# itmo153277/JoshUpscale

Hardware: AMD Instinct MI355X
Metric: frames/sec 480x270->1920x1080 recurrent SR (higher is better)
Workload: dtype bf16

## Files before the change

joshupscale_amd/csrc/c_api.cpp:

```cpp

#include "joshupscale_amd.h"
#ifdef JU_TEST_HOOKS
#include "joshupscale_amd_test.h"
#endif

#include <cstdio>
#include <cstring>
#include <fstream>
#include <ios>
#include <new>
#include <stdexcept>
#include <string>
#include <vector>

#include "engine.h"
#include "fp8.h"
#include "graphics.h"
#include "log.h"
#include "model.h"
#include "tiled.h"

struct ju_runtime {
	std::unique_ptr<ju::Engine> engine;
};
// ... 1452 lines not shown
}

int ju_debug_e4m3(const float *values, unsigned char *codes, size_t count) {
	return guarded([&] {
		if (count && (!values || !codes)) throw std::invalid_argument("ju_debug_e4m3: null buffer");
		for (size_t i = 0; i < count; ++i) codes[i] = ju::e4m3FromFloat(values[i]);
	});
}

}
namespace {

constexpr int kDebugAxisMax = 4096;

struct DebugRefuse {
	const char *hook;
	[[noreturn]] void operator()(const std::string &why) const { throw std::invalid_argument(std::string(hook) + ": " + why); }
};

bool misaligned(const void *p, std::uintptr_t a) { return reinterpret_cast<std::uintptr_t>(p) % a != 0; }

ju::DType debugDType(const DebugRefuse &refuse, int dtype) {
	if (dtype != JU_DTYPE_F16 && dtype != JU_DTYPE_BF16) refuse("dtype must be JU_DTYPE_F16 or JU_DTYPE_BF16");
	return dtype == JU_DTYPE_F16 ? ju::kF16 : ju::kBF16;
}

void debugActivation(const DebugRefuse &refuse, int act, float slope) {
	if (act < 0 || act > 2) refuse("an activation code outside 0 .. 2");
	if (act == 2 && !(slope >= 0.0f && slope <= 1.0f)) refuse("a LeakyReLU slope outside [0, 1]");
}

ju::DevPlan debugPlan(const DebugRefuse &refuse, const ju_debug_plan &p, ju::PlanLog *log) {
	if (p.flow_tile < 0 || p.res_block < 0 || p.res_block > 2 || p.conv_stages < -1 || p.conv_stages > 2 || p.splitk_rows < 0 ||
	    p.splitk_blocks < 0 || p.splitk_blocks > 2 || p.conv_nb < 0 || p.conv_nb > 2 || p.conv_rw < 0 || p.conv_rw > 2) {
		refuse("a plan field out of range");
	}
	ju::DevPlan plan;
	plan.flowTile = p.flow_tile;
	plan.resBlock = p.res_block;
	plan.convStages = p.conv_stages;
	plan.splitkRows = p.splitk_rows;
	plan.splitkBlocks = p.splitk_blocks;
	plan.convNb = p.conv_nb;
	plan.convRw = p.conv_rw;
	plan.log = log;
	return plan;
}

void debugPlanText(const ju::PlanLog &log, char *dst, std::size_t capacity) {
	if (dst == nullptr || capacity == 0) return;
	const std::string text = log.text();
	const std::size_t n = std::min(text.size(), capacity - 1);
	std::memcpy(dst, text.data(), n);
	dst[n] = '\0';
}

ju::DeviceBuffer debugPackWeights(const float *w, int taps, int cinReal, int cinPadded, int cout, int nb, ju::DType dt) {
	ju::FoldedConv conv;
	conv.taps = taps;
	conv.cin = cinReal;
	conv.cout = cout;
	conv.w.assign(w, w + static_cast<std::size_t>(taps) * cinReal * cout);
	std::vector<int> cinMap(static_cast<std::size_t>(cinPadded), -1);
	for (int c = 0; c < cinReal; ++c) cinMap[static_cast<std::size_t>(c)] = c;
	const std::vector<std::uint16_t> packed = ju::packConvWeights(conv, cinMap, nb, dt);
	ju::DeviceBuffer dev(packed.size() * 2);
	dev.upload(packed.data(), packed.size() * 2);
	return dev;
}

ju::DeviceBuffer debugUploadBias(const float *bias, int cout) {
	ju::DeviceBuffer dev(static_cast<std::size_t>(cout) * 4);
	dev.upload(bias, static_cast<std::size_t>(cout) * 4);
	return dev;
}

void debugPitch(const DebugRefuse &refuse, int pitch, int width, const char *what) {
// ... 362 lines not shown
```

joshupscale_amd/csrc/dev_switch.cpp:

```cpp
#include "dev_switch.h"

#ifdef JU_TEST_HOOKS
#include <cstddef>
#include <cstdlib>
#endif

namespace ju {

#ifdef JU_TEST_HOOKS
const char *devSwitch(Dev which) {
	static const char *const kNames[] = {
	    "JU_TAIL", "JU_PACK", "JU_POOL", "JU_UPSAMPLE", "JU_FLOW_CONV", "JU_TOWER", "JU_CALIBRATE", "JU_FLOW", "JU_DIRECT",
	    "JU_DIRECT_GRAPH", "JU_SYNC_SPIN_US", "JU_TRACE_STEPS", "JU_TRACE_NOSYNC", "JU_RES_BLOCK", "JU_FLOW_TILE",
	    "JU_FLOW_WIDE", "JU_WAVE_PRIO", "JU_CONV_DBUF", "JU_TOWER_FAST", "JU_FP8_GRID", "JU_FP8_BLOCK", "JU_SPLITK_PLAN",
	    "JU_CONV_TILE",
	};
	static_assert(sizeof(kNames) / sizeof(kNames[0]) == static_cast<std::size_t>(Dev::Count),
	    "kNames must name every switch of Dev, in its order");
	const int i = static_cast<int>(which);
	if (i < 0 || i >= static_cast<int>(Dev::Count)) return nullptr;
	return std::getenv(kNames[i]);
}
bool devSwitchesExist() {
	return true;
}
#else
const char *devSwitch(Dev) {
	return nullptr;
}
bool devSwitchesExist() {
	return false;
}
#endif

}
```

joshupscale_amd/csrc/dev_switch.h:

```cpp
#pragma once

namespace ju {

enum class Dev : int {
	Tail,
	Pack,
	Pool,
	Upsample,
	FlowConv,
	Tower,
	Calibrate,
	Flow,
	Direct,
	DirectGraph,
	SyncSpinUs,
	TraceSteps,
	TraceNoSync,
	ResBlock,
	FlowTile,
	FlowWide,
	WavePrio,
	ConvDbuf,
	TowerFast,
	Fp8Grid,
	Fp8Block,
	SplitKPlan,
	ConvTile,
	Count
};

const char *devSwitch(Dev which);
bool devSwitchesExist();

}
```

joshupscale_amd/csrc/engine.cpp:

```cpp
#include "engine.h"

#include <cstdio>

#include <algorithm>
#include <atomic>
#include <cstdlib>
#include <cstring>
#include <memory>
#include <mutex>
#include <sstream>
#include <stdexcept>

#include "dev_switch.h"
#include "fp8.h"
#include "graphics.h"
#include "log.h"

namespace ju {

namespace {
thread_local int g_DryLaunches = 0;
}
bool launchesAreDry() { return g_DryLaunches > 0; }
DryLaunchScope::DryLaunchScope() { ++g_DryLaunches; }
// ... 175 lines not shown
			throw std::invalid_argument("fp8 tower needs a 64-filter generator with at least one residual block");
		}
		m_Fp8Tower = true;
		dt = kF16;
	}
	if (dt != kF16 && dt != kBF16) throw std::invalid_argument("Unsupported compute dtype");
	m_DType = static_cast<DType>(dt);
	readSwitches();
	planFlowUnits();
	buildWeights(model);
	setUpResidentTowers();
	allocateBuffers(model);
	buildProgram(0);
	buildProgram(1);
	bindStaging();
	warmUpAndCapture();
}

namespace {
bool switchIs(Dev which, const char *word) {
	const char *v = devSwitch(which);
	return v && std::string(v) == word;
}
}

void Engine::readSwitches() {
	m_FusedTail = !switchIs(Dev::Tail, "split");
	m_TailInTower = !switchIs(Dev::Tail, "fused") && !switchIs(Dev::Tail, "split");
	m_PackInBlock = !switchIs(Dev::Pack, "split");
	m_FusedPool = !switchIs(Dev::Pool, "split");
	m_FusedUpsample = !switchIs(Dev::Upsample, "split");
	m_FlowFused = !switchIs(Dev::FlowConv, "generic");
	if (const char *e = devSwitch(Dev::FlowTile)) m_Plan.flowTile = std::atoi(e);
	if (const char *e = devSwitch(Dev::ResBlock)) m_Plan.resBlock = std::string(e) == "plain" ? 1 : (std::string(e) == "tile" ? 2 : 0);
	if (const char *e = devSwitch(Dev::ConvDbuf)) m_Plan.convStages = (e[0] >= '0' && e[0] <= '2') ? e[0] - '0' : -1;
	if (const char *e = devSwitch(Dev::SplitKPlan)) {
		m_Plan.splitkRows = std::atoi(e);
		if (const char *x = std::strchr(e, 'x')) m_Plan.splitkBlocks = std::atoi(x + 1);
	}
	if (const char *e = devSwitch(Dev::ConvTile)) {
		m_Plan.convNb = std::atoi(e);
		if (const char *x = std::strchr(e, 'x')) m_Plan.convRw = std::atoi(x + 1);
	}
	if (devSwitchesExist()) m_Plan.log = &m_PlanLog;
	const char *direct = devSwitch(Dev::Direct);
	m_PreferDirect = !(direct && direct[0] == '0');
	if (const char *retry = std::getenv("JU_RESIDENT_RETRY")) m_RetryBase = static_cast<unsigned>(std::atoi(retry));
	const char *directGraph = devSwitch(Dev::DirectGraph);
	m_DirectGraph = !(directGraph && directGraph[0] == '0');
	if (const char *spin = devSwitch(Dev::SyncSpinUs)) m_SpinUs = static_cast<unsigned>(std::atoi(spin));
	if (const char *la = std::getenv("JU_LOOKAHEAD")) m_BatchMax = std::min(std::max(std::atoi(la), 1), kFlowBatchMax);
}

bool Engine::setUpResidentTower(ResidentTower *t, bool wanted, int H, int W, int cus, bool leaky) {
	const bool on = wanted && residentTowerGeometry(H, W, cus, &t->GX, &t->GY, &t->RH);
	if (on) {
		t->w = DeviceBuffer(t->hostW.size() * 2);
		t->w.upload(t->hostW.data(), t->hostW.size() * 2);
		t->b = DeviceBuffer(t->hostB.size() * 4);
		t->b.upload(t->hostB.data(), t->hostB.size() * 4);
		const bool eightBit = m_Fp8Tower && t == &m_GenTower;
		t->mail = DeviceBuffer(eightBit ? residentMailboxBytes8(t->GX, t->GY, leaky) : residentMailboxBytes(t->GX, t->GY, leaky));
		t->flags = DeviceBuffer(residentCounterBytes(t->GX, t->GY));
	}
	t->hostW.clear();
	t->hostW.shrink_to_fit();
// ... 712 lines not shown
```

joshupscale_amd/csrc/flow_block_common.h:

```cpp
#pragma once

#include "kernel_common.h"

namespace ju {

void launchResBlockPersistent(DType dt, const FlowBlockLaunch &q, hipStream_t stream);

namespace {

constexpr int kFbW = 34;
constexpr int kFbOutW = 30;

__device__ __forceinline__ void fbGlds16(const void *g, void *l) {
	__builtin_amdgcn_global_load_lds((const __attribute__((address_space(1))) void *)g,
	    (__attribute__((address_space(3))) void *)l, 16, 0, 0);
}

template <int PB>
__device__ __forceinline__ unsigned fbSwz(unsigned col) {
	if constexpr (PB == 256) return col & 15u;
	else if constexpr (PB == 128) return (col >> 1) & 7u;
	else if constexpr (PB == 64) return (col >> 2) & 3u;
	else return (col >> 3) & 1u;
}

template <typename T, int KS, int PB>
struct FbPair {
	static constexpr int RS = kFbW * PB;
	static constexpr int NMAC = 3 * KS;

	template <int J>
	static __device__ __forceinline__ void rd(Vec8<T> &dst, unsigned a) {
		asm volatile("ds_read_b128 %0, %1 offset:%2" : "=v"(dst) : "v"(a), "n"(RS * J));
	}
	template <int ROT = 0>
	static __device__ __forceinline__ void issue(Vec8<T> (&fb)[4], unsigned rowAddr,
	    const unsigned (&colOff)[3], const unsigned (&colSwz)[3], int hh, int m, int j) {
		const int dx = m / KS, ks = m % KS;
		const unsigned a = rowAddr + colOff[dx] + ((static_cast<unsigned>(ks * 2 + hh) ^ colSwz[dx]) << 4);
		if (j == 0) rd<(0 + ROT) % 4>(fb[0], a);
		else if (j == 1) rd<(1 + ROT) % 4>(fb[1], a);
		else if (j == 2) rd<(2 + ROT) % 4>(fb[2], a);
		else rd<(3 + ROT) % 4>(fb[3], a);
	}
	template <int N>
	static __device__ __forceinline__ void waitLgkm() {
		static_assert(N >= 0 && N <= 4, "lgkmcnt");
		if constexpr (N == 4) asm volatile("s_waitcnt lgkmcnt(4)" ::: "memory");
		else if constexpr (N == 3) asm volatile("s_waitcnt lgkmcnt(3)" ::: "memory");
		else if constexpr (N == 2) asm volatile("s_waitcnt lgkmcnt(2)" ::: "memory");
		else if constexpr (N == 1) asm volatile("s_waitcnt lgkmcnt(1)" ::: "memory");
		else asm volatile("s_waitcnt lgkmcnt(0)" ::: "memory");
	}

	template <int ROT = 0>
	static __device__ __forceinline__ void run(unsigned rowAddr, const unsigned (&colOff)[3],
	    const unsigned (&colSwz)[3], int hh, const Vec8<T> (&w)[9 * KS], f32x16 (&acc)[2]) {
		Vec8<T> fb[2][4];
		asm volatile("s_waitcnt lgkmcnt(0)" ::: "memory");
		__builtin_amdgcn_sched_barrier(0);
#pragma unroll
		for (int j = 0; j < 4; ++j) issue<ROT>(fb[0], rowAddr, colOff, colSwz, hh, 0, j);
#pragma unroll
		for (int m = 0; m < NMAC; ++m) {
			const int set = m & 1;
			const bool more = m + 1 < NMAC;
			const int dx = m / KS, ks = m % KS;
#pragma unroll
			for (int k = 0; k < 6; ++k) {
				const int dy = k >> 1, r = k & 1;
				const int need = r + dy;
				const bool fresh = k == 0 || k == 1 || k == 3 || k == 5;
				if (fresh) {
					const int allowed = (3 - need) + (more ? (k < 4 ? k : 4) : 0);
					if (allowed >= 4) waitLgkm<4>();
					else if (allowed == 3) waitLgkm<3>();
					else if (allowed == 2) waitLgkm<2>();
					else if (allowed == 1) waitLgkm<1>();
					else waitLgkm<0>();
					__builtin_amdgcn_sched_barrier(0);
				}
				acc[r] = mfma32(w[(dy * 3 + dx) * KS + ks], fb[set][need], acc[r]);
				if (more && k < 4) issue<ROT>(fb[set ^ 1], rowAddr, colOff, colSwz, hh, m + 1, k);
				__builtin_amdgcn_sched_barrier(0);
			}
		}
	}
};


__device__ __forceinline__ float fbActS(int act, float slope) {
	return act == 1 ? 0.0f : (act == 2 ? slope : 1.0f);
}
__device__ __forceinline__ float fbAct(float v, float s) {
	return v < 0.0f ? v * s : v;
}

__device__ __forceinline__ float fbSwapPair(float v) {
	return __builtin_bit_cast(float, __builtin_amdgcn_mov_dpp(__builtin_bit_cast(int, v), 0xB1, 0xF, 0xF, true));
}

}

}
```

joshupscale_amd/csrc/flow_kernels.hip:

```cpp
#include "flow_block_common.h"

namespace ju {

namespace {

struct FlowBlockParams {
	const void *in;
	const void *w1;
	const float *b1;
	const void *w2;
	const float *b2;
	void *out;
	int H, W;
	int inPitch, outPitch;
	int act1, act2;
	float slope;
	int skip;
	int prio;
	const void *packPrev;
	void *packOut;
	int frameH, frameW, padTop, padLeft, numInputs;
	const unsigned *sums;
	long inItem, outItem;
	const std::uint8_t *frames[kFlowBatchMax];
// ... 12 lines not shown
	static constexpr int XR = TH + 4;
	static constexpr int TR = TH + 2;
	static constexpr int XPLANE = XR * kFbW * PBX;
	static constexpr int PBT = CMID * 2;
	static constexpr int KS2 = CMID / 16;
	static constexpr int NCB = CMID / 32;
	static constexpr int TBYTES = TR * kFbW * PBT;
	static constexpr int LR = XR / 2 + 1, LC = kFbW / 2 + 1;
	static constexpr int LBYTES = UPS ? NPL * LR * LC * PBX : 0;
	static constexpr bool XPAIR = UPS && NPL > 2 && TH > 2;
	static constexpr int NPLX = XPAIR ? 2 : NPL;
	static constexpr int OFF_X = 0;
	static constexpr int OFF_T = NPLX * XPLANE;
	static constexpr int TREGION = TBYTES > LBYTES ? TBYTES : LBYTES;
	static constexpr int ESZ = 2;
	static constexpr int RBW = 32 * ESZ;
	static constexpr int STAGE_PX = POOL ? 16 : 64;
	static constexpr int STAGE_WAVE = STAGE_PX * RBW;
	static constexpr bool STAGE_IN_X = NPLX * XPLANE >= NW * STAGE_WAVE;
	static constexpr int OFF_STAGE = STAGE_IN_X ? OFF_X : OFF_T + TREGION;
	static constexpr int LDS = OFF_T + TREGION + (STAGE_IN_X ? 0 : NW * STAGE_WAVE);
	static_assert(CIN == 16 || CIN == 32 || CIN == 64 || CIN == 128 || CIN == 256, "input channels");
#ifndef JU_FB_RELOAD_MIN
#define JU_FB_RELOAD_MIN 3
#endif
	static constexpr bool RELOAD = NPL >= JU_FB_RELOAD_MIN;
	static_assert(CMID == 32 || CMID == 64 || CMID == 128, "block filters");
	static_assert(NW % NCB == 0, "cout blocks over the waves");
	static_assert(TH % 2 == 0 && TH >= 2, "row pairs");
	static constexpr bool FITS = LDS <= 160 * 1024;
};

template <typename T, int CIN, int CMID, int TH, bool UPS, bool POOL, int OUTK, int NW, bool PACK = false, bool INDEP = false,
    bool CUT = false>
__global__ __launch_bounds__(NW * 64, NW / 4) void flow_block_kernel(FlowBlockParams p) {
	static_assert(!PACK || (CIN == 16 && !UPS), "PACK: the 16-channel flow input");
	static_assert(!INDEP || PACK, "INDEP: a form of the input packing");
	static_assert(!CUT || (PACK && !INDEP), "CUT: a form of the look-ahead input packing");
	using G = FbGeom<CIN, CMID, TH, UPS, POOL, OUTK, NW>;
	constexpr int NT = NW * 64;
	extern __shared__ __attribute__((aligned(16))) unsigned char smem[];
	const int tid = threadIdx.x;
	const int wave = tid >> 6;
	if constexpr (NW == 8) applyWavePriority(p.prio, wave, NW);
	const int lane = tid & 63;
	const int px = lane & 31;
	const int hh = lane >> 5;
	const int x0 = blockIdx.x * kFbOutW;
	const int y0 = blockIdx.y * TH;
	const int item = blockIdx.z;
	const T *__restrict__ in = reinterpret_cast<const T *>(static_cast<const unsigned char *>(p.in) + item * p.inItem);
	const unsigned ldsBase = static_cast<unsigned>(reinterpret_cast<unsigned long long>(
	    (__attribute__((address_space(3))) unsigned char *)smem));

	constexpr int NCB = G::NCB;
	const int cb = wave % NCB;
	const int pstart = wave / NCB;
	constexpr int PSTEP = NW / NCB;
	const float s1 = fbActS(p.act1, p.slope), s2 = fbActS(p.act2, p.slope);

	constexpr int NWA = G::RELOAD ? ((NW == 4 && !G::XPAIR) ? 2 : 1) : G::NPL;
	Vec8<T> wa[NWA][9 * G::KS1];
	const unsigned char *waSrc = static_cast<const unsigned char *>(p.w1) +
	                             (size_t)cb * G::NPL * (9 * G::KS1 * 1024) + lane * 16;
	auto loadPlaneA = [&](int set, int pl) __attribute__((always_inline)) {
#pragma unroll
		for (int f = 0; f < 9 * G::KS1; ++f) {
			wa[set][f] = *reinterpret_cast<const Vec8<T> *>(waSrc + (size_t)(pl * 9 * G::KS1 + f) * 1024);
		}
	};
	if constexpr (G::RELOAD) {
		loadPlaneA(0, 0);
	} else {
#pragma unroll
		for (int pl = 0; pl < G::NPL; ++pl) loadPlaneA(pl, pl);
	}

	[[maybe_unused]] constexpr int LPPX = G::PBX / 16;
	[[maybe_unused]] auto expandPlanes = [&](int plFirst, int plCount) __attribute__((always_inline)) {
		if constexpr (UPS) {
			constexpr int LPP = LPPX;
			constexpr int NPIX = G::LR * G::LC;
			const unsigned char *smL = smem + G::OFF_T;
			constexpr int BR = G::XR / 2, BC = kFbW / 2;
			const int nel = plCount * BR * BC * LPP;
			for (int e = tid; e < nel; e += NT) {
				const int c = e % LPP;
				const int bq = (e / LPP) % (BR * BC);
				const int pl = plFirst + e / (LPP * BR * BC);
				const int br = bq / BC, bc = bq - br * BC;
				const unsigned char *base = smL + pl * (NPIX * G::PBX) + (br * G::LC + bc) * G::PBX + c * 16;
				const Vec8<T> tl = *reinterpret_cast<const Vec8<T> *>(base);
				const Vec8<T> tr = *reinterpret_cast<const Vec8<T> *>(base + G::PBX);
				const Vec8<T> bl = *reinterpret_cast<const Vec8<T> *>(base + G::LC * G::PBX);
				const Vec8<T> brr = *reinterpret_cast<const Vec8<T> *>(base + (G::LC + 1) * G::PBX);
				Vec8<T> o01, o10, o11;
#pragma unroll
				for (int j = 0; j < 8; ++j) {
					const float a = static_cast<float>(tl[j]), b2 = static_cast<float>(tr[j]);
					const float d = static_cast<float>(bl[j]), e2 = static_cast<float>(brr[j]);
					const float top = a + (b2 - a) * 0.5f;
					const float bot = d + (e2 - d) * 0.5f;
					o01[j] = static_cast<T>(top);
					o10[j] = static_cast<T>(a + (d - a) * 0.5f);
					o11[j] = static_cast<T>(top + (bot - top) * 0.5f);
				}
				const int r = 2 * br, k = 2 * bc;
				const int gy = y0 - 2 + r, gx = x0 - 2 + k;
				const Vec8<T> zero = {static_cast<T>(0.f), static_cast<T>(0.f), static_cast<T>(0.f), static_cast<T>(0.f),
// ... 167 lines not shown
			for (int g = 0; g < 4; ++g) biasA[g] = *reinterpret_cast<const f32x4 *>(p.b1 + cb * 32 + 8 * g + 4 * hh);
		}
		auto initAcc = [&](f32x16(&a)[2]) {
#pragma unroll
			for (int g = 0; g < 4; ++g) {
				f32x4 bg;
				if constexpr (kHoistBiasA) bg = biasA[g];
				else bg = *reinterpret_cast<const f32x4 *>(p.b1 + cb * 32 + 8 * g + 4 * hh);
#pragma unroll
				for (int r = 0; r < 2; ++r) {
#pragma unroll
					for (int i = 0; i < 4; ++i) a[r][4 * g + i] = bg[i];
				}
			}
		};
		auto epilogueA = [&](const f32x16(&a)[2], int pair) {
			const int gx = x0 - 1 + px;
			const bool colIn = gx >= 0 && gx < p.W;
#pragma unroll
			for (int r = 0; r < 2; ++r) {
				const int tr = 2 * pair + r;
				const int gy = y0 - 1 + tr;
				const float keep = (colIn && gy >= 0 && gy < p.H) ? 1.0f : 0.0f;
				unsigned char *row = smem + G::OFF_T + tr * (kFbW * G::PBT);
#pragma unroll
				for (int g = 0; g < 4; ++g) {
					*reinterpret_cast<Vec4<T> *>(row + tOff[g]) =
					    pack4<T>(fbAct(a[r][4 * g + 0], s1) * keep, fbAct(a[r][4 * g + 1], s1) * keep,
					        fbAct(a[r][4 * g + 2], s1) * keep, fbAct(a[r][4 * g + 3], s1) * keep);
				}
			}
		};
		if (JU_SKIP(p) & 2) {
		} else if constexpr (G::NPL == 1) {
			for (int pair = pstart; pair < NPAIR; pair += PSTEP) {
				initAcc(acc[0]);
				FbPair<T, G::KS1, G::PBX>::run(ldsBase + G::OFF_X + (2 * pair) * (kFbW * G::PBX), colOffA, colSwzA,
				    hh, wa[0], acc[0]);
				epilogueA(acc[0], pair);
			}
		} else {
#pragma unroll
			for (int s = 0; s < HOLD; ++s) initAcc(acc[s]);
#pragma unroll
			for (int pl = 0; pl < G::NPL; ++pl) {
				if constexpr (G::RELOAD && NWA == 2) {
					if (pl + 1 < G::NPL) loadPlaneA((pl + 1) & 1, pl + 1);
				}
				if constexpr (G::XPAIR) {
					if (pl + 1 < G::NPL && !(JU_SKIP(p) & 1)) expandPlanes(pl + 1, 1);
				}
#pragma unroll
				for (int s = 0; s < HOLD; ++s) {
					const int pair = pstart + s * PSTEP;
					if (pair < NPAIR) {
						FbPair<T, G::KS1, G::PBX>::run(
						    ldsBase + G::OFF_X + (G::XPAIR ? (pl & 1) : pl) * G::XPLANE + (2 * pair) * (kFbW * G::PBX), colOffA,
						    colSwzA, hh, wa[G::RELOAD ? (pl & (NWA - 1)) : pl], acc[s]);
					}
				}
				if constexpr (G::RELOAD && NWA == 1) {
					if (pl + 1 < G::NPL) loadPlaneA(0, pl + 1);
				}
				if constexpr (G::XPAIR) __syncthreads();
			}
#pragma unroll
			for (int s = 0; s < HOLD; ++s) {
				const int pair = pstart + s * PSTEP;
				if (pair < NPAIR) epilogueA(acc[s], pair);
			}
		}
	}

	Vec8<T> wb[9 * G::KS2];
	f32x4 biasB[4];
	{
		const unsigned char *wsrc = static_cast<const unsigned char *>(p.w2) + (size_t)cb * (9 * G::KS2 * 1024) + lane * 16;
#pragma unroll
		for (int f = 0; f < 9 * G::KS2; ++f) {
			constexpr int KSP = G::KS2 > 4 ? 4 : G::KS2;
			const int tap = f / G::KS2, ks = f % G::KS2;
			wb[f] = *reinterpret_cast<const Vec8<T> *>(wsrc + (size_t)(((ks / KSP) * 9 + tap) * KSP + ks % KSP) * 1024);
		}
#pragma unroll
		for (int g = 0; g < 4; ++g) biasB[g] = *reinterpret_cast<const f32x4 *>(p.b2 + cb * 32 + 8 * g + 4 * hh);
	}
	__syncthreads();

	unsigned colOffB[3], colSwzB[3];
#pragma unroll
	for (int dx = 0; dx < 3; ++dx) {
		colOffB[dx] = (px + dx) * G::PBT;
		colSwzB[dx] = fbSwz<G::PBT>(px + dx);
	}
	unsigned char *stage = smem + G::OFF_STAGE + wave * G::STAGE_WAVE;
	constexpr int NCH = G::RBW / 16;
	for (int pair = pstart; pair < ((JU_SKIP(p) & 4) ? 0 : TH / 2); pair += PSTEP) {
		f32x16 acc[2];
#pragma unroll
		for (int g = 0; g < 4; ++g) {
#pragma unroll
			for (int r = 0; r < 2; ++r) {
#pragma unroll
				for (int i = 0; i < 4; ++i) acc[r][4 * g + i] = biasB[g][i];
			}
		}
		FbPair<T, G::KS2, G::PBT>::run(ldsBase + G::OFF_T + (2 * pair) * (kFbW * G::PBT), colOffB, colSwzB, hh, wb, acc);
		Vec4<T> resv[2][4];
		if constexpr (OUTK == 2) {
			static_assert(CIN == CMID && !UPS && !POOL, "residual block: same width in and out");
#pragma unroll
			for (int r = 0; r < 2; ++r) {
				const int gy = min(y0 + 2 * pair + r, p.H - 1), gx = min(x0 + px, p.W - 1);
				const T *rp = in + ((size_t)gy * p.inPitch + gx) * CIN + cb * 32 + 4 * hh;
#pragma unroll
				for (int g = 0; g < 4; ++g) resv[r][g] = *reinterpret_cast<const Vec4<T> *>(rp + 8 * g);
			}
		}
		if constexpr (POOL) {
			const int pp = px >> 1;
#pragma unroll
			for (int g = 0; g < 4; ++g) {
				float v[4];
#pragma unroll
				for (int i = 0; i < 4; ++i) {
					float m = fmaxf(acc[0][4 * g + i], acc[1][4 * g + i]);
					m = fmaxf(m, fbSwapPair(m));
					v[i] = fbAct(m, s2);
				}
				if ((g >> 1) == (px & 1)) {
					const unsigned c = static_cast<unsigned>(g) ^ (static_cast<unsigned>(pp) & (NCH - 1));
					*reinterpret_cast<Vec4<T> *>(stage + pp * G::RBW + (c << 4) + hh * 8) = pack4<T>(v[0], v[1], v[2], v[3]);
				}
			}
		} else {
#pragma unroll
			for (int r = 0; r < 2; ++r) {
				const int pi = r * 32 + px;
#pragma unroll
				for (int g = 0; g < 4; ++g) {
// ... 11 lines not shown
						*reinterpret_cast<Vec4<T> *>(stage + pi * G::RBW + (c << 4) + hh * 8) = pack4<T>(v[0], v[1], v[2], v[3]);
					}
				}
			}
		}
		__builtin_amdgcn_fence(__ATOMIC_RELEASE, "wavefront");
		__builtin_amdgcn_wave_barrier();
		__builtin_amdgcn_fence(__ATOMIC_ACQUIRE, "wavefront");
		{
			unsigned char *outp = static_cast<unsigned char *>(p.out) + item * p.outItem;
			constexpr int PXI = 64 / NCH;
#pragma unroll
			for (int it = 0; it < G::STAGE_PX / PXI; ++it) {
				const int pi = it * PXI + lane / NCH;
				const unsigned slot = static_cast<unsigned>(lane % NCH);
				const unsigned chunk = slot ^ (static_cast<unsigned>(pi) & (NCH - 1));
				const uint4 val = *reinterpret_cast<const uint4 *>(stage + pi * G::RBW + (slot << 4));
				if (JU_SKIP(p) & 8) {
				} else if constexpr (POOL) {
					const int oy = (y0 >> 1) + pair, ox = (x0 >> 1) + pi;
					if (pi < kFbOutW / 2 && oy < (p.H >> 1) && ox < (p.W >> 1)) {
						*reinterpret_cast<uint4 *>(outp + (((size_t)oy * p.outPitch + ox) * CMID + cb * 32) * G::ESZ + chunk * 16) = val;
					}
				} else {
					const int gy = y0 + 2 * pair + (pi >> 5), gx = x0 + (pi & 31);
					if ((pi & 31) < kFbOutW && gy < p.H && gx < p.W) {
						*reinterpret_cast<uint4 *>(outp + (((size_t)gy * p.outPitch + gx) * CMID + cb * 32) * G::ESZ + chunk * 16) = val;
					}
				}
			}
		}
		__builtin_amdgcn_fence(__ATOMIC_RELEASE, "wavefront");
		__builtin_amdgcn_wave_barrier();
	}
}

template <int CIN, int CMID = 32>
constexpr int fbWaves() {
#if JU_FB_RELOAD_MIN <= 2
	if (CIN == 128 && CMID <= 64) return 8;
#endif
	return (CIN > 64 || CMID > 64) ? 4 : 8;
}

template <typename T, int CIN, int CMID, int TH, bool UPS, bool POOL, int OUTK, bool PACK = false, bool INDEP = false, bool CUT = false>
void launchFlowBlockInst(const FlowBlockParams &p, int items, hipStream_t stream) {
	constexpr int NW = fbWaves<CIN, CMID>();
	using G = FbGeom<CIN, CMID, TH, UPS, POOL, OUTK, NW>;
	static_assert(G::FITS, "tile does not fit LDS");
	auto kern = flow_block_kernel<T, CIN, CMID, TH, UPS, POOL, OUTK, NW, PACK, INDEP, CUT>;
	static std::atomic<std::uint64_t> ldsDone{0};
	ensureDynamicLds(reinterpret_cast<const void *>(kern), G::LDS, &ldsDone, "flow block");
	if (launchesAreDry()) return;
	dim3 grid((p.W + kFbOutW - 1) / kFbOutW, (p.H + TH - 1) / TH, items);
	hipLaunchKernelGGL(kern, grid, dim3(NW * 64), G::LDS, stream, p);
	hipCheckLaunch("flow_block");
}

constexpr int kFbMid = 14;
constexpr int kFbFixedRows = 8;

inline long fbLaunchCost(int H, long tilesX, int TH, int numCUs, int items = 1) {
	const long tiles = tilesX * ((H + TH - 1) / TH) * items;
	return (tiles + numCUs - 1) / numCUs * (TH + kFbFixedRows);
}

void fbNotePlan(const DevPlan *plan, int cin, int cmid, bool ups, bool pool, int outk, bool pack, bool indep, int H, int W,
    int items, int rows, const int *heights, int nHeights) {
	std::string line = "flow_block cin=" + std::to_string(cin) + " cmid=" + std::to_string(cmid) + " ups=" + std::to_string(ups) +
	                   " pool=" + std::to_string(pool) + " outk=" + std::to_string(outk) + " pack=" + std::to_string(pack) +
	                   " indep=" + std::to_string(indep) + " H=" + std::to_string(H) + " W=" + std::to_string(W) +
	                   " items=" + std::to_string(items) + " rows=" + std::to_string(rows) + " heights=";
	for (int i = 0; i < nHeights; ++i) line += (i ? "," : "") + std::to_string(heights[i]);
	plan->log->note(line);
}

template <typename T, int CIN, int CMID, bool UPS, bool POOL, int OUTK, bool PACK, bool INDEP, bool CUT, int... THS>
void launchFlowBlockBest(const FlowBlockParams &p, int items, int numCUs, const DevPlan *plan, hipStream_t stream) {
	const long tilesX = (p.W + kFbOutW - 1) / kFbOutW;
	const int forced = plan ? plan->flowTile : 0;
	int best = 0;
	long bestCost = 0;
	int heights[sizeof...(THS)], nHeights = 0;
	auto consider = [&](int TH, bool fits) {
		if (!fits) return;
		heights[nHeights++] = TH;
		const long c = forced == TH ? -1 : fbLaunchCost(p.H, tilesX, TH, numCUs, items);
		if (best == 0 || c < bestCost) {
			best = TH;
			bestCost = c;
		}
	};
	(consider(THS, FbGeom<CIN, CMID, THS, UPS, POOL, OUTK, fbWaves<CIN, CMID>()>::FITS), ...);
	if (plan && plan->log) fbNotePlan(plan, CIN, CMID, UPS, POOL, OUTK, PACK, INDEP, p.H, p.W, items, best, heights, nHeights);
	bool done = false;
	auto launch = [&](auto thTag) {
		constexpr int TH = decltype(thTag)::value;
		if constexpr (FbGeom<CIN, CMID, TH, UPS, POOL, OUTK, fbWaves<CIN, CMID>()>::FITS) {
			if (!done && best == TH) {
				launchFlowBlockInst<T, CIN, CMID, TH, UPS, POOL, OUTK, PACK, INDEP, CUT>(p, items, stream);
				done = true;
			}
		}
	};
	(launch(std::integral_constant<int, THS>{}), ...);
	if (!done) throw std::logic_error("flow block: no tile height fits");
}

template <typename T, int CIN, int CMID, bool UPS, bool POOL, int OUTK, bool PACK = false, bool INDEP = false, bool CUT = false>
void launchFlowBlockT(const FlowBlockParams &p, int items, int numCUs, const DevPlan *plan, hipStream_t stream) {
	if constexpr (OUTK == 2) {
		launchFlowBlockBest<T, CIN, CMID, UPS, POOL, OUTK, PACK, INDEP, CUT, kFbMid, 6>(p, items, numCUs, plan, stream);
	} else if constexpr (CMID == 128) {
		launchFlowBlockBest<T, CIN, CMID, UPS, POOL, OUTK, PACK, INDEP, CUT, 6, 4, 2>(p, items, numCUs, plan, stream);
	} else {
		launchFlowBlockBest<T, CIN, CMID, UPS, POOL, OUTK, PACK, INDEP, CUT, 20, 18, 10, 6>(p, items, numCUs, plan, stream);
	}
}

template <typename T>
void launchFlowBlockDT(const FlowBlockLaunch &q, hipStream_t stream) {
	FlowBlockParams p{};
	p.in = q.in;
	p.w1 = q.w1;
	p.b1 = q.b1;
	p.w2 = q.w2;
	p.b2 = q.b2;
	p.out = q.out;
	p.H = q.H;
	p.W = q.W;
	p.inPitch = q.inPitch ? q.inPitch : (q.upsample ? q.W / 2 : q.W);
	p.outPitch = q.outPitch ? q.outPitch : (q.pool ? q.W / 2 : q.W);
	p.act1 = q.act1;
	p.act2 = q.act2;
	p.slope = q.slope;
	p.skip = ablationSkipBits();
	p.prio = wavePriorityMode(0);
	p.packPrev = q.packPrev;
	p.packOut = q.packOut;
// ... 94 lines not shown
```

joshupscale_amd/csrc/kernels.h:

```cpp
#pragma once

#include <hip/hip_runtime_api.h>

#include <cstddef>
#include <cstdint>
#include <mutex>
#include <stdexcept>
#include <string>
#include <vector>

#include "tile_geometry.h"

namespace ju {

enum DType : int { kF16 = 0, kBF16 = 1 };

inline std::size_t dtypeSize(DType) { return 2; }

class PlanLog {
public:
	void note(const std::string &line) {
		std::lock_guard<std::mutex> lock(m_Mutex);
		for (const std::string &l : m_Lines) {
			if (l == line) return;
		}
		m_Lines.push_back(line);
	}
	std::string text() const {
		std::lock_guard<std::mutex> lock(m_Mutex);
		std::string out;
		for (const std::string &l : m_Lines) out += l + "\n";
		return out;
	}

private:
	mutable std::mutex m_Mutex;
	std::vector<std::string> m_Lines;
};
struct DevPlan {
	int flowTile = 0;
	int resBlock = 0;
	int convStages = -1;
	int splitkRows = 0;
	int splitkBlocks = 0;
	int convNb = 0;
	int convRw = 0;
	PlanLog *log = nullptr;
};

struct ConvParams {
	const void *in;
	const void *wgt;
	const float *bias;
	const void *res;
	void *out;
	int H, W;
	int cin, cout;
	int taps;
	int relu;
	float slope;
	int outHead;
	int pool;
	int upsample;
	int stages;
	int inPitch, outPitch, resPitch;
	int nb, rw;
	int items;
	long inItemBytes, outItemBytes;
	const DevPlan *plan;
};

inline int towerPitch(int W) { return (W + 31) / 32 * 32 + 2; }
inline int towerRows(int H) { return (H + 7) / 8 * 8 + 2; }
// ... 545 lines not shown
```

joshupscale_amd/runtime.py:

```python

from __future__ import annotations

import ctypes as C
import os
from typing import Optional, Tuple

import numpy as np

_LIB_NAME = "libJoshUpscale.so"
_TEST_LIB_NAME = "libJoshUpscale_test.so"
_LIBS: dict = {}

LOC_CPU, LOC_DEVICE, LOC_GRAPHICS_RESOURCE = 0, 1, 2
DTYPE_DEFAULT, DTYPE_F16, DTYPE_BF16 = -1, 0, 1
DTYPE_FP8 = 2
DTYPE_NAMES = {DTYPE_F16: "fp16", DTYPE_BF16: "bf16", DTYPE_FP8: "fp8"}


class JuImage(C.Structure):
    _fields_ = [("ptr", C.c_void_p), ("location", C.c_uint8),
                ("stride", C.c_ssize_t), ("width", C.c_size_t),
                ("height", C.c_size_t)]


# ... 121 lines not shown
def tiled_alpha_problem(mode: int, filter: int, src_width: int, src_height: int, out_width: int = 0, out_height: int = 0) -> str:
    if (out_width, out_height) == (0, 0):
        out_width, out_height = 4 * src_width, 4 * src_height
    return alpha_problem(mode, filter, src_width, src_height, out_width, out_height)


LOG_CALLBACK = C.CFUNCTYPE(None, C.c_char_p, C.c_int, C.c_char_p, C.c_void_p)


class JoshUpscaleError(RuntimeError):
    def __init__(self, code: int, message: str):
        super().__init__(f"[{code}] {message}")
        self.code = code
        self.message = message


class JuSceneInfo(C.Structure):
    _fields_ = [("step", C.c_uint64), ("sad", C.c_uint64), ("score", C.c_uint64), ("cut", C.c_uint32),
                ("reserved", C.c_uint32)]


SCENE_OFF, SCENE_REPORT, SCENE_RESET = 0, 1, 2
SCENE_RING = 64


class JuTiledInfo(C.Structure):
    _fields_ = [("src_width", C.c_size_t), ("src_height", C.c_size_t), ("out_width", C.c_size_t),
                ("out_height", C.c_size_t), ("tile_width", C.c_size_t), ("tile_height", C.c_size_t),
                ("tiles_x", C.c_int), ("tiles_y", C.c_int), ("overlap", C.c_int)]


class JuDebugPlan(C.Structure):
    _fields_ = [(n, C.c_int) for n in ("flow_tile", "res_block", "conv_stages", "splitk_rows", "splitk_blocks", "conv_nb",
                                       "conv_rw")]


class JuDebugConv(C.Structure):
    _fields_ = [("kernel", C.c_int), ("dtype", C.c_int), ("inp", C.c_void_p), ("res", C.c_void_p), ("out", C.c_void_p),
                ("weights", C.c_void_p), ("bias", C.c_void_p)] + \
               [(n, C.c_int) for n in ("H", "W", "cin", "cin_real", "cout", "taps", "relu")] + [("slope", C.c_float)] + \
               [(n, C.c_int) for n in ("out_head", "pool", "upsample", "nb", "rw", "in_pitch", "out_pitch", "res_pitch", "items")] + \
               [("in_item_bytes", C.c_longlong), ("out_item_bytes", C.c_longlong), ("plan", JuDebugPlan),
                ("plan_text", C.c_void_p), ("plan_capacity", C.c_size_t)]


class JuDebugFlowBlock(C.Structure):
    _fields_ = [("dtype", C.c_int), ("inp", C.c_void_p), ("out", C.c_void_p), ("weights1", C.c_void_p), ("bias1", C.c_void_p),
                ("weights2", C.c_void_p), ("bias2", C.c_void_p)] + \
               [(n, C.c_int) for n in ("H", "W", "cin", "cin_real", "cmid", "upsample", "pool", "out_head", "residual", "act1",
                                       "act2")] + [("slope", C.c_float)] + \
               [(n, C.c_int) for n in ("in_pitch", "out_pitch", "items")] + \
               [("in_item_bytes", C.c_longlong), ("out_item_bytes", C.c_longlong), ("plan", JuDebugPlan),
                ("plan_text", C.c_void_p), ("plan_capacity", C.c_size_t)]


class JuDebugResample(C.Structure):
    _fields_ = [("op", C.c_int), ("dtype", C.c_int), ("inp", C.c_void_p), ("out", C.c_void_p)] + \
               [(n, C.c_int) for n in ("H", "W", "C", "items")]


class JuDebugWarp(C.Structure):
    _fields_ = [("dtype", C.c_int), ("state", C.c_void_p), ("flow", C.c_void_p), ("frame", C.c_void_p),
                ("frame_stride", C.c_ssize_t), ("out", C.c_void_p)] + \
               [(n, C.c_int) for n in ("out_pitch", "H", "W", "PW", "pad_top", "pad_left")] + \
               [("sums", C.c_void_p), ("pre_warp_out", C.c_void_p), ("out_u8", C.c_void_p), ("out_stride", C.c_ssize_t)]


# ... 882 lines not shown
```

Baseline: 2156.

## Stream flow-block weights into registers behind the MFMA loop

Adds a STREAM variant of the flow block kernel for the one-wave-per-SIMD, 64-channel-plane shapes. It issues buffer loads for the next plane's conv-A weights and for conv-B weights inside the last pair's MAC loop, instead of bulk-loading them up front or between stages. The aim is to hide global weight-load latency behind matrix math. The cost is extra register pressure and more complex scheduling. It is on by default, and JU_FLOW_WSTREAM=0 or the plan's flow_burst field restores the old burst loads.

After: 2171 (median of 6 runs). Within noise of the previous version (+0.7%).

```diff
diff --git a/joshupscale_amd/csrc/c_api.cpp b/joshupscale_amd/csrc/c_api.cpp
--- a/joshupscale_amd/csrc/c_api.cpp
+++ b/joshupscale_amd/csrc/c_api.cpp
@@ -1508,7 +1508,8 @@
 
 ju::DevPlan debugPlan(const DebugRefuse &refuse, const ju_debug_plan &p, ju::PlanLog *log) {
 	if (p.flow_tile < 0 || p.res_block < 0 || p.res_block > 2 || p.conv_stages < -1 || p.conv_stages > 2 || p.splitk_rows < 0 ||
-	    p.splitk_blocks < 0 || p.splitk_blocks > 2 || p.conv_nb < 0 || p.conv_nb > 2 || p.conv_rw < 0 || p.conv_rw > 2) {
+	    p.splitk_blocks < 0 || p.splitk_blocks > 2 || p.conv_nb < 0 || p.conv_nb > 2 || p.conv_rw < 0 || p.conv_rw > 2 ||
+	    p.flow_burst < 0 || p.flow_burst > 1) {
 		refuse("a plan field out of range");
 	}
 	ju::DevPlan plan;
@@ -1519,6 +1520,7 @@
 	plan.splitkBlocks = p.splitk_blocks;
 	plan.convNb = p.conv_nb;
 	plan.convRw = p.conv_rw;
+	plan.flowBurst = p.flow_burst;
 	plan.log = log;
 	return plan;
 }
diff --git a/joshupscale_amd/csrc/dev_switch.cpp b/joshupscale_amd/csrc/dev_switch.cpp
--- a/joshupscale_amd/csrc/dev_switch.cpp
+++ b/joshupscale_amd/csrc/dev_switch.cpp
@@ -13,7 +13,7 @@
 	    "JU_TAIL", "JU_PACK", "JU_POOL", "JU_UPSAMPLE", "JU_FLOW_CONV", "JU_TOWER", "JU_CALIBRATE", "JU_FLOW", "JU_DIRECT",
 	    "JU_DIRECT_GRAPH", "JU_SYNC_SPIN_US", "JU_TRACE_STEPS", "JU_TRACE_NOSYNC", "JU_RES_BLOCK", "JU_FLOW_TILE",
 	    "JU_FLOW_WIDE", "JU_WAVE_PRIO", "JU_CONV_DBUF", "JU_TOWER_FAST", "JU_FP8_GRID", "JU_FP8_BLOCK", "JU_SPLITK_PLAN",
-	    "JU_CONV_TILE",
+	    "JU_CONV_TILE", "JU_FLOW_WSTREAM",
 	};
 	static_assert(sizeof(kNames) / sizeof(kNames[0]) == static_cast<std::size_t>(Dev::Count),
 	    "kNames must name every switch of Dev, in its order");
diff --git a/joshupscale_amd/csrc/dev_switch.h b/joshupscale_amd/csrc/dev_switch.h
--- a/joshupscale_amd/csrc/dev_switch.h
+++ b/joshupscale_amd/csrc/dev_switch.h
@@ -26,6 +26,7 @@
 	Fp8Block,
 	SplitKPlan,
 	ConvTile,
+	FlowWStream,
 	Count
 };
 
diff --git a/joshupscale_amd/csrc/engine.cpp b/joshupscale_amd/csrc/engine.cpp
--- a/joshupscale_amd/csrc/engine.cpp
+++ b/joshupscale_amd/csrc/engine.cpp
@@ -231,6 +231,7 @@
 	m_FusedUpsample = !switchIs(Dev::Upsample, "split");
 	m_FlowFused = !switchIs(Dev::FlowConv, "generic");
 	if (const char *e = devSwitch(Dev::FlowTile)) m_Plan.flowTile = std::atoi(e);
+	if (const char *e = devSwitch(Dev::FlowWStream)) m_Plan.flowBurst = std::atoi(e) == 0 ? 1 : 0;
 	if (const char *e = devSwitch(Dev::ResBlock)) m_Plan.resBlock = std::string(e) == "plain" ? 1 : (std::string(e) == "tile" ? 2 : 0);
 	if (const char *e = devSwitch(Dev::ConvDbuf)) m_Plan.convStages = (e[0] >= '0' && e[0] <= '2') ? e[0] - '0' : -1;
 	if (const char *e = devSwitch(Dev::SplitKPlan)) {
diff --git a/joshupscale_amd/csrc/flow_block_common.h b/joshupscale_amd/csrc/flow_block_common.h
--- a/joshupscale_amd/csrc/flow_block_common.h
+++ b/joshupscale_amd/csrc/flow_block_common.h
@@ -53,9 +53,12 @@
 		else asm volatile("s_waitcnt lgkmcnt(0)" ::: "memory");
 	}
 
-	template <int ROT = 0>
+	struct NoStream {
+		__device__ __forceinline__ void operator()(int) const {}
+	};
+	template <int ROT = 0, typename Behind = NoStream>
 	static __device__ __forceinline__ void run(unsigned rowAddr, const unsigned (&colOff)[3],
-	    const unsigned (&colSwz)[3], int hh, const Vec8<T> (&w)[9 * KS], f32x16 (&acc)[2]) {
+	    const unsigned (&colSwz)[3], int hh, const Vec8<T> (&w)[9 * KS], f32x16 (&acc)[2], Behind behind = Behind{}) {
 		Vec8<T> fb[2][4];
 		asm volatile("s_waitcnt lgkmcnt(0)" ::: "memory");
 		__builtin_amdgcn_sched_barrier(0);
@@ -84,6 +87,10 @@
 				if (more && k < 4) issue<ROT>(fb[set ^ 1], rowAddr, colOff, colSwz, hh, m + 1, k);
 				__builtin_amdgcn_sched_barrier(0);
 			}
+			if constexpr (!std::is_same<Behind, NoStream>::value) {
+				behind(m);
+				__builtin_amdgcn_sched_barrier(0);
+			}
 		}
 	}
 };
diff --git a/joshupscale_amd/csrc/flow_kernels.hip b/joshupscale_amd/csrc/flow_kernels.hip
--- a/joshupscale_amd/csrc/flow_kernels.hip
+++ b/joshupscale_amd/csrc/flow_kernels.hip
@@ -68,12 +68,13 @@
 };
 
 template <typename T, int CIN, int CMID, int TH, bool UPS, bool POOL, int OUTK, int NW, bool PACK = false, bool INDEP = false,
-    bool CUT = false>
+    bool CUT = false, bool STREAM = false>
 __global__ __launch_bounds__(NW * 64, NW / 4) void flow_block_kernel(FlowBlockParams p) {
 	static_assert(!PACK || (CIN == 16 && !UPS), "PACK: the 16-channel flow input");
 	static_assert(!INDEP || PACK, "INDEP: a form of the input packing");
 	static_assert(!CUT || (PACK && !INDEP), "CUT: a form of the look-ahead input packing");
 	using G = FbGeom<CIN, CMID, TH, UPS, POOL, OUTK, NW>;
+	static_assert(!STREAM || (NW == 4 && !G::XPAIR && !PACK && OUTK != 2), "STREAM: the one-wave-per-SIMD forms");
 	constexpr int NT = NW * 64;
 	extern __shared__ __attribute__((aligned(16))) unsigned char smem[];
 	const int tid = threadIdx.x;
@@ -105,12 +106,63 @@
 			wa[set][f] = *reinterpret_cast<const Vec8<T> *>(waSrc + (size_t)(pl * 9 * G::KS1 + f) * 1024);
 		}
 	};
-	if constexpr (G::RELOAD) {
+	auto undefinedSet = [&](Vec8<T>(&w)[9 * G::KS1]) __attribute__((always_inline)) {
+#pragma unroll
+		for (int f = 0; f < 9 * G::KS1; ++f) asm volatile("" : "=v"(w[f]));
+	};
+	if constexpr (G::RELOAD || STREAM) {
 		loadPlaneA(0, 0);
+		if constexpr (NWA == 2 && !STREAM) {
+			if (JU_SKIP(p) & 16) undefinedSet(wa[1]);
+		}
 	} else {
 #pragma unroll
-		for (int pl = 0; pl < G::NPL; ++pl) loadPlaneA(pl, pl);
-	}
+		for (int pl = 0; pl < G::NPL; ++pl) {
+			if (pl > 0 && (JU_SKIP(p) & 16)) undefinedSet(wa[pl]);
+			else loadPlaneA(pl, pl);
+		}
+	}
+
+	Vec8<T> wb[9 * G::KS2];
+	f32x4 biasB[4];
+	auto loadBiasB = [&]() __attribute__((always_inline)) {
+#pragma unroll
+		for (int g = 0; g < 4; ++g) biasB[g] = *reinterpret_cast<const f32x4 *>(p.b2 + cb * 32 + 8 * g + 4 * hh);
+	};
+	auto wbSource = [](int f) constexpr {
+		constexpr int KSP = G::KS2 > 4 ? 4 : G::KS2;
+		const int tap = f / G::KS2, ks = f % G::KS2;
+		return ((ks / KSP) * 9 + tap) * KSP + ks % KSP;
+	};
+	constexpr int kSetA = 9 * G::KS1, kSetB = 9 * G::KS2;
+	[[maybe_unused]] const __amdgpu_buffer_rsrc_t rsrcWa =
+	    __builtin_amdgcn_make_buffer_rsrc(const_cast<void *>(p.w1), 0, NCB * G::NPL * kSetA * 1024, 0x00020000);
+	[[maybe_unused]] const __amdgpu_buffer_rsrc_t rsrcWb =
+	    __builtin_amdgcn_make_buffer_rsrc(const_cast<void *>(p.w2), 0, NCB * kSetB * 1024, 0x00020000);
+	[[maybe_unused]] const unsigned waLane = static_cast<unsigned>(cb * (G::NPL * kSetA * 1024) + lane * 16);
+	[[maybe_unused]] const unsigned wbLane = static_cast<unsigned>(cb * (kSetB * 1024) + lane * 16);
+	[[maybe_unused]] auto streamA = [&](int set, int pl, int f) __attribute__((always_inline)) {
+		if (JU_SKIP(p) & 16) asm volatile("" : "=v"(wa[set][f]));
+		else wa[set][f] = __builtin_bit_cast(Vec8<T>, __builtin_amdgcn_raw_buffer_load_b128(rsrcWa, waLane, (pl * kSetA + f) * 1024, 0));
+	};
+	[[maybe_unused]] auto streamB = [&](int u) __attribute__((always_inline)) {
+		const int m = u / 3, dy = u % 3;
+		const int f = (dy * 3 + m / G::KS2) * G::KS2 + m % G::KS2;
+		if (JU_SKIP(p) & 32) asm volatile("" : "=v"(wb[f]));
+		else wb[f] = __builtin_bit_cast(Vec8<T>, __builtin_amdgcn_raw_buffer_load_b128(rsrcWb, wbLane, wbSource(f) * 1024, 0));
+	};
+	constexpr int kStreamSteps = (G::NPL > 1 && (G::TR / 2 + PSTEP - 1) / PSTEP >= 2 ? 2 : 1) * 3 * G::KS1;
+	constexpr int kFirstB = 36;
+	[[maybe_unused]] auto streamStepA = [&](int pl, int g) __attribute__((always_inline)) {
+		if (g >= kStreamSteps) return;
+#pragma unroll
+		for (int u = g * 36 / kStreamSteps; u < (g + 1) * 36 / kStreamSteps; ++u) {
+			const int m = u / 3, dy = u % 3;
+			if (pl + 1 < G::NPL) streamA(G::RELOAD ? ((pl + 1) & 1) : pl + 1, pl + 1, (dy * 3 + m / G::KS1) * G::KS1 + m % G::KS1);
+			else streamB(u);
+		}
+	};
+	static_assert(!STREAM || (kSetA == 36 && (NWA == 2 || G::NPL == 1)), "STREAM: 64-channel planes, two register sets");
 
 	[[maybe_unused]] constexpr int LPPX = G::PBX / 16;
 	[[maybe_unused]] auto expandPlanes = [&](int plFirst, int plCount) __attribute__((always_inline)) {
@@ -344,20 +396,36 @@
 			}
 		};
 		if (JU_SKIP(p) & 2) {
+			if constexpr (STREAM) {
+				loadBiasB();
+#pragma unroll
+				for (int u = 0; u < kFirstB; ++u) streamB(u);
+			}
 		} else if constexpr (G::NPL == 1) {
-			for (int pair = pstart; pair < NPAIR; pair += PSTEP) {
+			static_assert(!STREAM || PSTEP == 1, "STREAM: every wave runs every pair");
+			for (int pair = pstart; pair < (STREAM ? NPAIR - 1 : NPAIR); pair += PSTEP) {
 				initAcc(acc[0]);
 				FbPair<T, G::KS1, G::PBX>::run(ldsBase + G::OFF_X + (2 * pair) * (kFbW * G::PBX), colOffA, colSwzA,
 				    hh, wa[0], acc[0]);
 				epilogueA(acc[0], pair);
 			}
+			if constexpr (STREAM) {
+				loadBiasB();
+				initAcc(acc[0]);
+				FbPair<T, G::KS1, G::PBX>::run(ldsBase + G::OFF_X + (2 * (NPAIR - 1)) * (kFbW * G::PBX), colOffA, colSwzA,
+				    hh, wa[0], acc[0], [&](int m) __attribute__((always_inline)) { streamStepA(0, m); });
+				epilogueA(acc[0], NPAIR - 1);
+			}
 		} else {
 #pragma unroll
 			for (int s = 0; s < HOLD; ++s) initAcc(acc[s]);
 #pragma unroll
 			for (int pl = 0; pl < G::NPL; ++pl) {
-				if constexpr (G::RELOAD && NWA == 2) {
-					if (pl + 1 < G::NPL) loadPlaneA((pl + 1) & 1, pl + 1);
+				if constexpr (G::RELOAD && NWA == 2 && !STREAM) {
+					if (pl + 1 < G::NPL && !(JU_SKIP(p) & 16)) loadPlaneA((pl + 1) & 1, pl + 1);
+				}
+				if constexpr (STREAM) {
+					if (pl + 1 == G::NPL) loadBiasB();
 				}
 				if constexpr (G::XPAIR) {
 					if (pl + 1 < G::NPL && !(JU_SKIP(p) & 1)) expandPlanes(pl + 1, 1);
@@ -365,14 +433,24 @@
 #pragma unroll
 				for (int s = 0; s < HOLD; ++s) {
 					const int pair = pstart + s * PSTEP;
-					if (pair < NPAIR) {
+					if constexpr (STREAM) {
+						constexpr int NMACA = 3 * G::KS1;
+						if (pair < NPAIR) {
+							FbPair<T, G::KS1, G::PBX>::run(ldsBase + G::OFF_X + pl * G::XPLANE + (2 * pair) * (kFbW * G::PBX), colOffA,
+							    colSwzA, hh, wa[G::RELOAD ? (pl & 1) : pl], acc[s],
+							    [&](int m) __attribute__((always_inline)) { streamStepA(pl, s * NMACA + m); });
+						} else {
+#pragma unroll
+							for (int m = 0; m < NMACA; ++m) streamStepA(pl, s * NMACA + m);
+						}
+					} else if (pair < NPAIR) {
 						FbPair<T, G::KS1, G::PBX>::run(
 						    ldsBase + G::OFF_X + (G::XPAIR ? (pl & 1) : pl) * G::XPLANE + (2 * pair) * (kFbW * G::PBX), colOffA,
 						    colSwzA, hh, wa[G::RELOAD ? (pl & (NWA - 1)) : pl], acc[s]);
 					}
 				}
 				if constexpr (G::RELOAD && NWA == 1) {
-					if (pl + 1 < G::NPL) loadPlaneA(0, pl + 1);
+					if (pl + 1 < G::NPL && !(JU_SKIP(p) & 16)) loadPlaneA(0, pl + 1);
 				}
 				if constexpr (G::XPAIR) __syncthreads();
 			}
@@ -384,18 +462,14 @@
 		}
 	}
 
-	Vec8<T> wb[9 * G::KS2];
-	f32x4 biasB[4];
-	{
+	if constexpr (!STREAM) {
 		const unsigned char *wsrc = static_cast<const unsigned char *>(p.w2) + (size_t)cb * (9 * G::KS2 * 1024) + lane * 16;
 #pragma unroll
 		for (int f = 0; f < 9 * G::KS2; ++f) {
-			constexpr int KSP = G::KS2 > 4 ? 4 : G::KS2;
-			const int tap = f / G::KS2, ks = f % G::KS2;
-			wb[f] = *reinterpret_cast<const Vec8<T> *>(wsrc + (size_t)(((ks / KSP) * 9 + tap) * KSP + ks % KSP) * 1024);
-		}
-#pragma unroll
-		for (int g = 0; g < 4; ++g) biasB[g] = *reinterpret_cast<const f32x4 *>(p.b2 + cb * 32 + 8 * g + 4 * hh);
+			if (JU_SKIP(p) & 32) asm volatile("" : "=v"(wb[f]));
+			else wb[f] = *reinterpret_cast<const Vec8<T> *>(wsrc + (size_t)wbSource(f) * 1024);
+		}
+		loadBiasB();
 	}
 	__syncthreads();
 
@@ -407,7 +481,9 @@
 	}
 	unsigned char *stage = smem + G::OFF_STAGE + wave * G::STAGE_WAVE;
 	constexpr int NCH = G::RBW / 16;
-	for (int pair = pstart; pair < ((JU_SKIP(p) & 4) ? 0 : TH / 2); pair += PSTEP) {
+	constexpr bool kStreamB2 = STREAM && kSetB > kFirstB;
+	static_assert(!kStreamB2 || (PSTEP == 1 && kSetB == 2 * kFirstB), "STREAM: every wave has conv B's first pair");
+	auto pairB = [&](int pair, auto streamTag) __attribute__((always_inline)) {
 		f32x16 acc[2];
 #pragma unroll
 		for (int g = 0; g < 4; ++g) {
@@ -417,7 +493,17 @@
 				for (int i = 0; i < 4; ++i) acc[r][4 * g + i] = biasB[g][i];
 			}
 		}
-		FbPair<T, G::KS2, G::PBT>::run(ldsBase + G::OFF_T + (2 * pair) * (kFbW * G::PBT), colOffB, colSwzB, hh, wb, acc);
+		if constexpr (decltype(streamTag)::value) {
+			FbPair<T, G::KS2, G::PBT>::run(ldsBase + G::OFF_T + (2 * pair) * (kFbW * G::PBT), colOffB, colSwzB, hh, wb, acc,
+			    [&](int m) __attribute__((always_inline)) {
+				    if (m < kFirstB / 3) {
+#pragma unroll
+					    for (int dy = 0; dy < 3; ++dy) streamB(kFirstB + 3 * m + dy);
+				    }
+			    });
+		} else {
+			FbPair<T, G::KS2, G::PBT>::run(ldsBase + G::OFF_T + (2 * pair) * (kFbW * G::PBT), colOffB, colSwzB, hh, wb, acc);
+		}
 		Vec4<T> resv[2][4];
 		if constexpr (OUTK == 2) {
 			static_assert(CIN == CMID && !UPS && !POOL, "residual block: same width in and out");
@@ -495,6 +581,13 @@
 		}
 		__builtin_amdgcn_fence(__ATOMIC_RELEASE, "wavefront");
 		__builtin_amdgcn_wave_barrier();
+	};
+	const int npairB = (JU_SKIP(p) & 4) ? 0 : TH / 2;
+	if constexpr (kStreamB2) {
+		if (npairB > 0) pairB(pstart, std::true_type{});
+		for (int pair = pstart + PSTEP; pair < npairB; pair += PSTEP) pairB(pair, std::false_type{});
+	} else {
+		for (int pair = pstart; pair < npairB; pair += PSTEP) pairB(pair, std::false_type{});
 	}
 }
 
@@ -506,12 +599,19 @@
 	return (CIN > 64 || CMID > 64) ? 4 : 8;
 }
 
-template <typename T, int CIN, int CMID, int TH, bool UPS, bool POOL, int OUTK, bool PACK = false, bool INDEP = false, bool CUT = false>
+template <int CIN, int CMID, int TH, bool UPS, bool POOL, int OUTK, bool PACK>
+constexpr bool fbStreams() {
+	constexpr int NW = fbWaves<CIN, CMID>();
+	return NW == 4 && !FbGeom<CIN, CMID, TH, UPS, POOL, OUTK, NW>::XPAIR && !PACK && OUTK != 2;
+}
+
+template <typename T, int CIN, int CMID, int TH, bool UPS, bool POOL, int OUTK, bool PACK = false, bool INDEP = false, bool CUT = false,
+    bool STREAM = false>
 void launchFlowBlockInst(const FlowBlockParams &p, int items, hipStream_t stream) {
 	constexpr int NW = fbWaves<CIN, CMID>();
 	using G = FbGeom<CIN, CMID, TH, UPS, POOL, OUTK, NW>;
 	static_assert(G::FITS, "tile does not fit LDS");
-	auto kern = flow_block_kernel<T, CIN, CMID, TH, UPS, POOL, OUTK, NW, PACK, INDEP, CUT>;
+	auto kern = flow_block_kernel<T, CIN, CMID, TH, UPS, POOL, OUTK, NW, PACK, INDEP, CUT, STREAM>;
 	static std::atomic<std::uint64_t> ldsDone{0};
 	ensureDynamicLds(reinterpret_cast<const void *>(kern), G::LDS, &ldsDone, "flow block");
 	if (launchesAreDry()) return;
@@ -529,11 +629,11 @@
 }
 
 void fbNotePlan(const DevPlan *plan, int cin, int cmid, bool ups, bool pool, int outk, bool pack, bool indep, int H, int W,
-    int items, int rows, const int *heights, int nHeights) {
+    int items, int rows, bool stream, const int *heights, int nHeights) {
 	std::string line = "flow_block cin=" + std::to_string(cin) + " cmid=" + std::to_string(cmid) + " ups=" + std::to_string(ups) +
 	                   " pool=" + std::to_string(pool) + " outk=" + std::to_string(outk) + " pack=" + std::to_string(pack) +
 	                   " indep=" + std::to_string(indep) + " H=" + std::to_string(H) + " W=" + std::to_string(W) +
-	                   " items=" + std::to_string(items) + " rows=" + std::to_string(rows) + " heights=";
+	                   " items=" + std::to_string(items) + " rows=" + std::to_string(rows) + " stream=" + std::to_string(stream) + " heights=";
 	for (int i = 0; i < nHeights; ++i) line += (i ? "," : "") + std::to_string(heights[i]);
 	plan->log->note(line);
 }
@@ -555,12 +655,19 @@
 		}
 	};
 	(consider(THS, FbGeom<CIN, CMID, THS, UPS, POOL, OUTK, fbWaves<CIN, CMID>()>::FITS), ...);
-	if (plan && plan->log) fbNotePlan(plan, CIN, CMID, UPS, POOL, OUTK, PACK, INDEP, p.H, p.W, items, best, heights, nHeights);
-	bool done = false;
+	const bool burst = plan && plan->flowBurst;
+	bool done = false, streamed = false;
 	auto launch = [&](auto thTag) {
 		constexpr int TH = decltype(thTag)::value;
 		if constexpr (FbGeom<CIN, CMID, TH, UPS, POOL, OUTK, fbWaves<CIN, CMID>()>::FITS) {
 			if (!done && best == TH) {
+				if constexpr (fbStreams<CIN, CMID, TH, UPS, POOL, OUTK, PACK>()) {
+					if (!burst) {
+						launchFlowBlockInst<T, CIN, CMID, TH, UPS, POOL, OUTK, PACK, INDEP, CUT, true>(p, items, stream);
+						streamed = done = true;
+						return;
+					}
+				}
 				launchFlowBlockInst<T, CIN, CMID, TH, UPS, POOL, OUTK, PACK, INDEP, CUT>(p, items, stream);
 				done = true;
 			}
@@ -568,6 +675,7 @@
 	};
 	(launch(std::integral_constant<int, THS>{}), ...);
 	if (!done) throw std::logic_error("flow block: no tile height fits");
+	if (plan && plan->log) fbNotePlan(plan, CIN, CMID, UPS, POOL, OUTK, PACK, INDEP, p.H, p.W, items, best, streamed, heights, nHeights);
 }
 
 template <typename T, int CIN, int CMID, bool UPS, bool POOL, int OUTK, bool PACK = false, bool INDEP = false, bool CUT = false>
diff --git a/joshupscale_amd/csrc/kernels.h b/joshupscale_amd/csrc/kernels.h
--- a/joshupscale_amd/csrc/kernels.h
+++ b/joshupscale_amd/csrc/kernels.h
@@ -39,6 +39,7 @@
 };
 struct DevPlan {
 	int flowTile = 0;
+	int flowBurst = 0;
 	int resBlock = 0;
 	int convStages = -1;
 	int splitkRows = 0;
diff --git a/joshupscale_amd/runtime.py b/joshupscale_amd/runtime.py
--- a/joshupscale_amd/runtime.py
+++ b/joshupscale_amd/runtime.py
@@ -177,7 +177,7 @@
 
 class JuDebugPlan(C.Structure):
     _fields_ = [(n, C.c_int) for n in ("flow_tile", "res_block", "conv_stages", "splitk_rows", "splitk_blocks", "conv_nb",
-                                       "conv_rw")]
+                                       "conv_rw", "flow_burst")]
 
 
 class JuDebugConv(C.Structure):
```
